# COMP6248-Reproducability-Challenge/selfsupervised-denoising

Measured on AMD Instinct MI355X. Metric: training patches/sec (64x64 gauss25 SSDN), higher is better.
Workload: dtype f16

## Files before the change

### selfsupervised-denoising_amd/csrc/api.hip

```cpp
#include "common.h"
#include <cstdarg>
#include <cstdio>
#include <cstdlib>

static thread_local char g_err[512] = "";
thread_local hipEvent_t g_ssdn_stop_event = nullptr;
thread_local bool g_ssdn_stop_used = false;
thread_local hipEvent_t g_ssdn_prof_start = nullptr, g_ssdn_prof_stop = nullptr;
thread_local bool g_ssdn_prof_used = false;

int ssdn_set_error(const char* fmt, ...) {
    va_list ap;
    va_start(ap, fmt);
    vsnprintf(g_err, sizeof(g_err), fmt, ap);
    va_end(ap);
    return -1;
}

#include <vector>
struct ProfSlot {
    bool on = false;
    std::vector<hipEvent_t> ev;
    size_t used = 0;
    double flops = 0.0, bytes = 0.0;
// ... 203 lines not shown
                }
                SSDN_CHECK_HIP(hipStreamWaitEvent(lane_s[lane], cover[src], 0));
                dirty[src][lane] = false;
            }
        }
        const bool is_mark = ops[i].type == SSDN_OP_EVENT_RECORD;
        if (!is_mark) {
            for (int d = 0; d < SSDN_NLANES; ++d) dirty[lane][d] = true;
            covered[lane] = false;
        }
        used[lane] = true;
        hipStream_t s = lane_s[lane];
        bool armed = false;
        long long armed_at = 0;
        auto arm = [&](int j) {
            if (!has_side || no_stop || j >= n) return;
            const int lj = one_lane ? 0 : ops[j].lane;
            if (lj == lane || lj < 0 || lj >= SSDN_NLANES || !((g_lane_deps[lj] >> lane) & 1)) return;
            armed_at = LS->ev_next;
            g_ssdn_stop_event = LS->ev[LS->ev_next++ % SSDN_NEVENTS];
            g_ssdn_stop_used = false;
            armed = true;
        };
        auto arm_last = [&](int j) {
            if (!has_side || no_stop || lane == 0 || armed) return;
            for (; j < n; ++j)
                if ((one_lane ? 0 : ops[j].lane) == lane && ops[j].type != SSDN_OP_EVENT_RECORD) return;
            armed_at = LS->ev_next;
            g_ssdn_stop_event = LS->ev[LS->ev_next++ % SSDN_NEVENTS];
            g_ssdn_stop_used = false;
            armed = true;
        };
        switch (ops[i].type) {
            case SSDN_OP_PACK_INPUT: {
                const bool next_conv = i + 1 < n && ops[i + 1].type == SSDN_OP_CONV && ops[i + 1].args && (one_lane ? 0 : ops[i + 1].lane) == lane;
                if (next_conv && chain_merging_on() && conv_pack_fusable((const ssdn_pack_input_args*)p, (const ssdn_conv_args*)ops[i + 1].args)) {
                    rc = launch_conv_thin((const ssdn_conv_args*)ops[i + 1].args, (const ssdn_pack_input_args*)p, s);
                    ++i;
                } else rc = launch_pack_input((const ssdn_pack_input_args*)p, s);
                break;
            }
            case SSDN_OP_CONV: {
                const int m = chain_len(ops + i, n - i, one_lane);
                if (m < 0) return -1;
                const bool pair = m <= 1 && i + 1 < n && ops[i + 1].type == SSDN_OP_CONV && ops[i + 1].args && (one_lane ? 0 : ops[i + 1].lane) == lane &&
                                  chain_merging_on() && conv_pair_fusable((const ssdn_conv_args*)p, (const ssdn_conv_args*)ops[i + 1].args);
                arm(i + (m > 1 ? m : (pair ? 2 : 1)));
                if (m > 1) { rc = launch_chain(ops + i, m, one_lane, s); i += m - 1; }
                else if (pair) { rc = launch_gemm_dma_with_next((const ssdn_conv_args*)p, (const ssdn_conv_args*)ops[i + 1].args, s); ++i; }
                else rc = launch_conv((const ssdn_conv_args*)p, s);
                break;
            }
            case SSDN_OP_POOL_FWD: rc = launch_pool_fwd((const ssdn_pool_args*)p, s); break;
            case SSDN_OP_POOL_BWD: arm(i + 1); rc = launch_pool_bwd((const ssdn_pool_args*)p, s); break;
            case SSDN_OP_UPSUM_BWD: arm(i + 1); rc = launch_upsum_bwd((const ssdn_upsum_args*)p, s); break;
            case SSDN_OP_UNROT_FWD: rc = launch_unrot_fwd((const ssdn_unrot_args*)p, s); break;
            case SSDN_OP_UNROT_BWD: arm(i + 1); rc = launch_unrot_bwd((const ssdn_unrot_args*)p, s); break;
            case SSDN_OP_WGRAD: {
                static const bool no_merge = ssdn_tuning_env("SSDN_NO_WGRAD_MERGE") != nullptr;
                {
                    const ssdn_wgrad_args* mg[WGRAD_MEGA_MAX];
                    int mm = 0;
                    while (!no_merge && mm < WGRAD_MEGA_MAX && i + mm < n && ops[i + mm].type == SSDN_OP_WGRAD && ops[i + mm].args &&
                           (one_lane ? 0 : ops[i + mm].lane) == lane && wgrad_mega_ok((const ssdn_wgrad_args*)ops[i + mm].args) &&
                           ((const ssdn_wgrad_args*)ops[i + mm].args)->mega == ((const ssdn_wgrad_args*)p)->mega)
                        mg[mm] = (const ssdn_wgrad_args*)ops[i + mm].args, ++mm;
                    if (mm > 1) { arm(i + mm); rc = launch_wgrad_mega(mg, mm, s); i += mm - 1; break; }
                }
                const ssdn_wgrad_args* items[WGRAD_MULTI_MAX];
                int m = 0;
                while (!no_merge && m < WGRAD_MULTI_MAX && i + m < n && ops[i + m].type == SSDN_OP_WGRAD && ops[i + m].args &&
                       (one_lane ? 0 : ops[i + m].lane) == lane && wgrad_mergeable((const ssdn_wgrad_args*)ops[i + m].args))
                    items[m] = (const ssdn_wgrad_args*)ops[i + m].args, ++m;
                if (m > 1) { rc = launch_wgrad_multi(items, m, s); i += m - 1; }
                else rc = launch_wgrad((const ssdn_wgrad_args*)p, s);
                break;
            }
            case SSDN_OP_WREDUCE: {
                const ssdn_wreduce_args* items[WREDUCE_MULTI_MAX];
                int m = 0;
                while (m < WREDUCE_MULTI_MAX && i + m < n && ops[i + m].type == SSDN_OP_WREDUCE && ops[i + m].args &&
                       (one_lane ? 0 : ops[i + m].lane) == lane)
                    items[m] = (const ssdn_wreduce_args*)ops[i + m].args, ++m;
                arm_last(i + m);
                rc = m > 1 ? launch_wreduce_multi(items, m, s) : launch_wreduce((const ssdn_wreduce_args*)p, s);
                i += m - 1;
                break;
            }
            case SSDN_OP_WPACK: {
                const ssdn_wpack_args* items[WPACK_MULTI_MAX];
                int m = 0;
                while (m < WPACK_MULTI_MAX && i + m < n && ops[i + m].type == SSDN_OP_WPACK && ops[i + m].args &&
                       (one_lane ? 0 : ops[i + m].lane) == lane)
                    items[m] = (const ssdn_wpack_args*)ops[i + m].args, ++m;
                rc = m > 1 ? launch_wpack_multi(items, m, s) : launch_wpack((const ssdn_wpack_args*)p, s);
                i += m - 1;
                break;
            }
            case SSDN_OP_GRAD_PACK: {
                const bool next_conv = i + 1 < n && ops[i + 1].type == SSDN_OP_CONV && ops[i + 1].args && (one_lane ? 0 : ops[i + 1].lane) == lane;
                if (next_conv && chain_merging_on() && conv_gradpack_fusable((const ssdn_grad_pack_args*)p, (const ssdn_conv_args*)ops[i + 1].args)) {
                    arm(i + 2);
                    rc = launch_gradpack_dgrad((const ssdn_grad_pack_args*)p, (const ssdn_conv_args*)ops[i + 1].args, s);
                    ++i;
                } else { arm(i + 1); rc = launch_grad_pack((const ssdn_grad_pack_args*)p, s); }
                break;
            }
            case SSDN_OP_HEAD_SSDN: rc = launch_head((const ssdn_head_args*)p, s); break;
            case SSDN_OP_HEAD_FINAL: rc = launch_head_final((const ssdn_head_final_args*)p, s); break;
            case SSDN_OP_SPATIAL_MEAN: rc = launch_spatial_mean((const ssdn_spatial_mean_args*)p, s); break;
            case SSDN_OP_MSE: rc = launch_mse((const ssdn_mse_args*)p, 0, s); break;
            case SSDN_OP_MASK_MSE: rc = launch_mse((const ssdn_mse_args*)p, 1, s); break;
            case SSDN_OP_ADAM: {
                const ssdn_wpack_args* items[ADAM_PACK_MAX];
                int m = 0;
                while (m < ADAM_PACK_MAX && i + 1 + m < n && ops[i + 1 + m].type == SSDN_OP_WPACK && ops[i + 1 + m].args &&
                       (one_lane ? 0 : ops[i + 1 + m].lane) == lane)
                    items[m] = (const ssdn_wpack_args*)ops[i + 1 + m].args, ++m;
                const bool whole_run = !(i + 1 + m < n && ops[i + 1 + m].type == SSDN_OP_WPACK);
                if (m > 0 && whole_run && adam_pack_fusable((const ssdn_adam_args*)p, items, m)) {
                    rc = launch_adam_pack((const ssdn_adam_args*)p, items, m, s);
                    i += m;
                } else rc = launch_adam((const ssdn_adam_args*)p, s);
                break;
            }
            case SSDN_OP_METRICS: rc = launch_metrics((const ssdn_metrics_args*)p, s); break;
            case SSDN_OP_NOISE: rc = launch_noise((const ssdn_noise_args*)p, s); break;
            case SSDN_OP_INPUT_GRAD: arm(i + 1); rc = launch_input_grad((const ssdn_input_grad_args*)p, s); break;
            case SSDN_OP_HEAD_VJP: rc = launch_head_vjp((const ssdn_head_vjp_args*)p, s); break;
            case SSDN_OP_MSE_VJP: rc = launch_mse_vjp((const ssdn_mse_vjp_args*)p, s); break;
            case SSDN_OP_ACCUM: rc = launch_accum((const ssdn_accum_args*)p, s); break;
            case SSDN_OP_ZERO: {
                const ssdn_zero_args* z = (const ssdn_zero_args*)p;
                if (z->bytes & 15) return ssdn_set_error("op %d: zero size must be a multiple of 16", i);
                long long n16 = z->bytes / 16;
                int g = (int)((n16 + 255) / 256);
                if (g > 2048) g = 2048;
                if (g > 0) hipLaunchKernelGGL(k_zero, dim3(g), dim3(256), 0, s, (uint4*)z->p, n16);
                break;
            }
            case SSDN_OP_EVENT_RECORD: {
                const ssdn_event_args* e = (const ssdn_event_args*)p;
                if (!e->event) return ssdn_set_error("op %d: null event", i);
                SSDN_CHECK_HIP(hipEventRecord((hipEvent_t)e->event, s));
                break;
            }
            default: return ssdn_set_error("op %d: unknown type %d", i, ops[i].type);
        }
        if (armed) {
            if (g_ssdn_stop_used && !rc) { cover[lane] = g_ssdn_stop_event; covered[lane] = true; cover_at[lane] = armed_at; }
            g_ssdn_stop_event = nullptr;
        }
        if (rc) {
            char tmp[400];
            snprintf(tmp, sizeof(tmp), "%s", g_err);
            return ssdn_set_error("op %d (type %d): %s", i, ops[i].type, tmp);
        }
    }
    for (int l = 1; l < SSDN_NLANES; ++l) {
        if (!used[l]) continue;
        if (!cover_live(l)) {
            cover[l] = LS->ev[LS->ev_next++ % SSDN_NEVENTS];
            SSDN_CHECK_HIP(hipEventRecord(cover[l], lane_s[l]));
        }
        SSDN_CHECK_HIP(hipStreamWaitEvent(lane_s[0], cover[l], 0));
    }
// ... 41 lines not shown
```

### selfsupervised-denoising_amd/csrc/common.h

```cpp
#pragma once
#include <hip/hip_runtime.h>
#include <hip/hip_ext.h>
#include <stdint.h>
#include "../../include/ssdn_hip.h"
#include <cstdlib>

#if defined(SSDN_TUNING)
static inline const char* ssdn_tuning_env(const char* name) { return std::getenv(name); }
#else
static inline const char* ssdn_tuning_env(const char*) { return nullptr; }
#endif

typedef _Float16 h16;
typedef _Float16 half8 __attribute__((ext_vector_type(8)));
typedef _Float16 half4 __attribute__((ext_vector_type(4)));
typedef _Float16 half2v __attribute__((ext_vector_type(2)));
typedef __bf16 bf16x8 __attribute__((ext_vector_type(8)));
typedef unsigned short u16x8 __attribute__((ext_vector_type(8)));
typedef unsigned short u16x4 __attribute__((ext_vector_type(4)));
typedef float f32x16 __attribute__((ext_vector_type(16)));
typedef float f32x4 __attribute__((ext_vector_type(4)));

#define LRELU_SLOPE 0.1f

// ... 31 lines not shown
}
static __device__ __forceinline__ float bf_lo(unsigned w) { return __uint_as_float(w << 16); }
static __device__ __forceinline__ float bf_hi(unsigned w) { return __uint_as_float(w & 0xffff0000u); }
static __device__ __forceinline__ float f16_lo(unsigned w) { return (float)__builtin_bit_cast(f16x2_t, w)[0]; }
static __device__ __forceinline__ float f16_hi(unsigned w) { return (float)__builtin_bit_cast(f16x2_t, w)[1]; }
#define SSDN_BUFFER_RSRC_FLAGS 0x00020000
static __device__ __forceinline__ u16x8 ld_b8(const unsigned short* p) { return *reinterpret_cast<const u16x8*>(p); }
static __device__ __forceinline__ void st_b8(unsigned short* p, u16x8 v) { *reinterpret_cast<u16x8*>(p) = v; }
static __device__ __forceinline__ u16x4 ld_b4(const unsigned short* p) { return *reinterpret_cast<const u16x4*>(p); }
static __device__ __forceinline__ void st_b4(unsigned short* p, u16x4 v) { *reinterpret_cast<u16x4*>(p) = v; }
static __device__ __forceinline__ u16x8 zero_b8() {
    u16x8 z;
#pragma unroll
    for (int i = 0; i < 8; ++i) z[i] = 0;
    return z;
}

static __device__ __forceinline__ half8 zero_h8() {
    half8 z;
#pragma unroll
    for (int i = 0; i < 8; ++i) z[i] = (h16)0.f;
    return z;
}

extern thread_local hipEvent_t g_ssdn_stop_event;
extern thread_local bool g_ssdn_stop_used;
extern thread_local hipEvent_t g_ssdn_prof_start, g_ssdn_prof_stop;
extern thread_local bool g_ssdn_prof_used;
#define SSDN_LAUNCH(kernel, grid, block, lds, stream, ...)                                                                       \
    do {                                                                                                                         \
        if (g_ssdn_stop_event) {                                                                                                 \
            hipExtLaunchKernelGGL(kernel, grid, block, lds, stream, nullptr, g_ssdn_stop_event, 0, __VA_ARGS__);                 \
            g_ssdn_stop_used = true;                                                                                             \
        } else if (g_ssdn_prof_start) {                                                                                          \
            hipExtLaunchKernelGGL(kernel, grid, block, lds, stream, g_ssdn_prof_start, g_ssdn_prof_stop, 0, __VA_ARGS__);        \
            g_ssdn_prof_start = nullptr;                                                                                         \
            g_ssdn_prof_used = true;                                                                                             \
        } else hipLaunchKernelGGL(kernel, grid, block, lds, stream, __VA_ARGS__);                                                \
    } while (0)

#define SSDN_MAX_DEVICES_ATTR 16
static inline int ssdn_current_device_slot() {
    int dev = 0;
    if (hipGetDevice(&dev) != hipSuccess || dev < 0) dev = 0;
    return dev % SSDN_MAX_DEVICES_ATTR;
}

void prof_begin(int kind, hipStream_t s);
void prof_end(int kind, hipStream_t s, double flops, double bytes);

int launch_conv(const ssdn_conv_args* a, hipStream_t s);
int launch_wgrad(const ssdn_wgrad_args* a, hipStream_t s);
bool wgrad_mergeable(const ssdn_wgrad_args* a);
int launch_wgrad_multi(const ssdn_wgrad_args* const* items, int n, hipStream_t s);
#define WGRAD_MEGA_MAX 64
int wgrad_mega_ok(const ssdn_wgrad_args* a);
int launch_wgrad_mega(const ssdn_wgrad_args* const* ops, int n, hipStream_t s);
int launch_pack_input(const ssdn_pack_input_args* a, hipStream_t s);
int launch_pool_fwd(const ssdn_pool_args* a, hipStream_t s);
int launch_pool_bwd(const ssdn_pool_args* a, hipStream_t s);
int launch_upsum_bwd(const ssdn_upsum_args* a, hipStream_t s);
int launch_unrot_fwd(const ssdn_unrot_args* a, hipStream_t s);
int launch_unrot_bwd(const ssdn_unrot_args* a, hipStream_t s);
int launch_wreduce(const ssdn_wreduce_args* a, hipStream_t s);
int launch_wpack(const ssdn_wpack_args* a, hipStream_t s);
#define WPACK_MULTI_MAX 24
int launch_wpack_multi(const ssdn_wpack_args* const* items, int n, hipStream_t s);
#define WREDUCE_MULTI_MAX 32
#define WGRAD_MULTI_MAX 32
int launch_wreduce_multi(const ssdn_wreduce_args* const* items, int n, hipStream_t s);
int launch_grad_pack(const ssdn_grad_pack_args* a, hipStream_t s);
int launch_head(const ssdn_head_args* a, hipStream_t s);
int launch_head_impulse(const ssdn_head_args* a, hipStream_t s);
int launch_head_final(const ssdn_head_final_args* a, hipStream_t s);
int launch_spatial_mean(const ssdn_spatial_mean_args* a, hipStream_t s);
int launch_mse(const ssdn_mse_args* a, int masked, hipStream_t s);
int launch_head_vjp(const ssdn_head_vjp_args* a, hipStream_t s);
int launch_head_vjp_impulse(const ssdn_head_vjp_args* a, hipStream_t s);
int launch_mse_vjp(const ssdn_mse_vjp_args* a, hipStream_t s);
int launch_adam(const ssdn_adam_args* a, hipStream_t s);
#define ADAM_PACK_MAX 24
int adam_pack_fusable(const ssdn_adam_args* a, const ssdn_wpack_args* const* items, int n);
int launch_adam_pack(const ssdn_adam_args* a, const ssdn_wpack_args* const* items, int n, hipStream_t s);
int launch_metrics(const ssdn_metrics_args* a, hipStream_t s);
int launch_accum(const ssdn_accum_args* a, hipStream_t s);
int launch_noise(const ssdn_noise_args* a, hipStream_t s);
int launch_input_grad(const ssdn_input_grad_args* a, hipStream_t s);
int conv_lds_bytes(const ssdn_conv_args* a);
int conv_validate(const ssdn_conv_args* a);
int chain_len(const ssdn_op* ops, int n, bool any_lane);
int launch_chain(const ssdn_op* ops, int n, bool any_lane, hipStream_t s);
bool chain_merging_on();
bool conv_dma_eligible(const ssdn_conv_args* a, bool any_size);
int conv_dma_lds_bytes(int mt);
bool conv_signs(const ssdn_conv_args* a);
bool gemm_dma_signs(const ssdn_conv_args* a);
bool conv_dma_signs(const ssdn_conv_args* a);
bool conv_fuses_urot(const ssdn_conv_args* a);
bool conv_fuses_unrot(const ssdn_conv_args* a);
bool conv_fuses_upsum(const ssdn_conv_args* a);
bool conv_fuses_pool(const ssdn_conv_args* a);
int launch_conv_dma(const ssdn_conv_args* a, hipStream_t s);
bool conv_thin_eligible(const ssdn_conv_args* a);
bool conv_thin_fuses_pack(const ssdn_pack_input_args* pk, const ssdn_conv_args* a);
int launch_conv_thin(const ssdn_conv_args* a, const ssdn_pack_input_args* pk, hipStream_t s);
bool conv_pack_fusable(const ssdn_pack_input_args* pk, const ssdn_conv_args* a);
bool gradpack_dgrad_fusable(const ssdn_grad_pack_args* gp, const ssdn_conv_args* a);
int launch_gradpack_dgrad(const ssdn_grad_pack_args* gp, const ssdn_conv_args* a, hipStream_t s);
bool conv_gradpack_fusable(const ssdn_grad_pack_args* gp, const ssdn_conv_args* a);
bool gemm_dma_eligible(const ssdn_conv_args* a);
int gemm_dma_lds_bytes(const ssdn_conv_args* a);
int launch_gemm_dma(const ssdn_conv_args* a, hipStream_t s);
bool gemm_dma_fuses_next(const ssdn_conv_args* a, const ssdn_conv_args* b);
int launch_gemm_dma_with_next(const ssdn_conv_args* a, const ssdn_conv_args* b, hipStream_t s);
bool conv_pair_fusable(const ssdn_conv_args* a, const ssdn_conv_args* b);
extern "C" int ssdn_device_cus(void);
int wgrad_lds_bytes(const ssdn_wgrad_args* a);
```

### selfsupervised-denoising_amd/csrc/elementwise.hip

```cpp
#include "common.h"

#define EW_BLOCK 256
static inline int ew_grid(long long n) {
    long long g = (n + EW_BLOCK - 1) / EW_BLOCK;
    return (int)(g < 1 ? 1 : g);
}

__global__ void k_pack_input(ssdn_pack_input_args a) {
    const unsigned idx = blockIdx.x * blockDim.x + threadIdx.x;
    const int H = a.H, W = a.W;
    long long total = (long long)a.R * a.B * H * W;
    if (idx >= total) return;
    int j = idx % W;
    int i = (idx / W) % H;
    int nb = idx / (unsigned)(W * H);
    int r = nb / a.B, b = nb % a.B;
    int sy, sx;
    switch (r) {
        case 0: sy = i; sx = j; break;
        case 1: sy = j; sx = W - 1 - i; break;
        case 2: sy = H - 1 - i; sx = W - 1 - j; break;
        default: sy = H - 1 - j; sx = i; break;
    }
    h16* d = (h16*)a.dst.p + (long long)idx * a.dst.cs + a.dst.co;
    for (int c0 = 0; c0 < a.cpad; c0 += 8) {
        half8 v = zero_h8();
#pragma unroll
        for (int c = 0; c < 8; ++c)
            if (c0 + c < a.C) v[c] = (h16)a.src[(((long long)b * a.C + c0 + c) * H + sy) * W + sx];
        st_h8(d + c0, v);
    }
}
int launch_pack_input(const ssdn_pack_input_args* a, hipStream_t s) {
    if (a->R == 4 && a->H != a->W) return ssdn_set_error("pack_input: blind-spot rotation needs square images");
    long long n = (long long)a->R * a->B * a->H * a->W;
    if (n >= (1ll << 31)) return ssdn_set_error("pack_input: too many elements for 32-bit indexing");
    hipLaunchKernelGGL(k_pack_input, dim3(ew_grid(n)), dim3(EW_BLOCK), 0, s, *a);
    return 0;
}

__global__ void k_pool_fwd(ssdn_pool_args a) {
    const unsigned idx = blockIdx.x * blockDim.x + threadIdx.x;
    const int C8 = a.C >> 3, Ho = a.H >> 1, Wo = a.W >> 1;
    long long total = (long long)a.N * Ho * Wo * C8;
    if (idx >= total) return;
    int c = (idx % C8) * 8;
    const unsigned p = idx / C8;
    int j = p % Wo;
    int i = (p / Wo) % Ho;
    int n = p / (unsigned)(Wo * Ho);
    const h16* src = (const h16*)a.act.p + a.act.co + c;
    int r0 = a.shifted ? 2 * i - 1 : 2 * i;
    const bool padrow = a.shifted && r0 < 0;
    float m[8];
    unsigned win[8];
#pragma unroll
    for (int q = 0; q < 8; ++q) { m[q] = padrow ? 0.f : -65504.f; win[q] = 4u; }
#pragma unroll
    for (int dr = 0; dr < 2; ++dr) {
        int y = r0 + dr;
        if (y < 0) continue;
#pragma unroll
        for (int dc = 0; dc < 2; ++dc) {
            half8 v = ld_h8(src + (((long long)n * a.H + y) * a.W + 2 * j + dc) * a.act.cs);
#pragma unroll
            for (int q = 0; q < 8; ++q) {
                const float f = (float)v[q];
                if (f > m[q] || (!padrow && dr == 0 && dc == 0)) win[q] = (unsigned)(2 * dr + dc);
                m[q] = fmaxf(m[q], f);
            }
        }
    }
    half8 o;
#pragma unroll
    for (int q = 0; q < 8; ++q) o[q] = (h16)m[q];
    st_h8((h16*)a.pooled.p + a.pooled.co + c + (((long long)n * Ho + i) * Wo + j) * a.pooled.cs, o);
    if (a.route) {
        unsigned r = 0;
#pragma unroll
        for (int q = 0; q < 8; ++q) r |= (win[q] | (m[q] > 0.f ? 8u : 0u)) << (4 * q);
        ((unsigned*)a.route)[idx] = r;
    }
}
// ... 416 lines not shown
        t1.bstart[i] = b1;
        t2.bstart[i] = b2;
        if (a->nslabs > WR_GROUP) {
            t1.gx[i] = ew_grid(stride / 4);
            b1 += t1.gx[i] * ((a->nslabs + WR_GROUP - 1) / WR_GROUP);
            t2.step[i] = WR_GROUP;
        } else {
            t1.gx[i] = 0;
            t2.step[i] = 1;
        }
        t1.step[i] = t2.step[i];
        t2.gx[i] = t1.gx[i];
        if (a->Kpad & 3) return ssdn_set_error("wreduce: Kpad must be a multiple of 4");
        b2 += ew_grid(stride / 4 + a->M);
    }
    t1.bstart[n] = b1;
    t2.bstart[n] = b2;
    if (b1 > 0) hipLaunchKernelGGL(k_wreduce_partial_multi, dim3(b1), dim3(EW_BLOCK), 0, s, t1);
    if (b2 > 0) SSDN_LAUNCH(k_wreduce_multi, dim3(b2), dim3(EW_BLOCK), 0, s, t2);
    return 0;
}

int launch_wreduce(const ssdn_wreduce_args* a, hipStream_t s) {
    long long stride = (long long)a->ntaps * a->Mpad * a->Kpad;
    int step = 1;
    if (a->nslabs > WR_GROUP) {
        int groups = (a->nslabs + WR_GROUP - 1) / WR_GROUP;
        hipLaunchKernelGGL(k_wreduce_partial, dim3(ew_grid(stride / 4), groups), dim3(EW_BLOCK), 0, s, (float*)a->slab, stride, a->nslabs);
        step = WR_GROUP;
    }
    if (a->Kpad & 3) return ssdn_set_error("wreduce: Kpad must be a multiple of 4");
    long long n = stride / 4 + a->M;
    SSDN_LAUNCH(k_wreduce, dim3(ew_grid(n)), dim3(EW_BLOCK), 0, s, *a, step);
    return 0;
}

__global__ void k_accum(ssdn_accum_args a) {
    const long long i = (long long)blockIdx.x * blockDim.x + threadIdx.x;
    if (i < a.n) a.dst[i] = __fadd_rn(a.dst[i], a.src[i]);
}
int launch_accum(const ssdn_accum_args* a, hipStream_t s) {
    if (!a->dst || !a->src || a->n < 0) return ssdn_set_error("accum: dst and src must be given, n >= 0");
    if (a->n > 0) hipLaunchKernelGGL(k_accum, dim3(ew_grid(a->n)), dim3(EW_BLOCK), 0, s, *a);
    return 0;
}

struct AdamIn { float g, m, v, p; };
static __device__ __forceinline__ AdamIn adam_load(const ssdn_adam_args& a, long long i) { return AdamIn{a.g[i], a.m[i], a.v[i], a.p[i]}; }
static __device__ __forceinline__ float adam_apply(const ssdn_adam_args& a, long long i, const AdamIn& q, float inv_bc2s, float step) {
    const float g = q.g * a.gscale;
    const float m = __fmaf_rn(a.b1, q.m, __fmul_rn(1.f - a.b1, g));
    const float v = __fmaf_rn(a.b2, q.v, __fmul_rn(__fmul_rn(1.f - a.b2, g), g));
    a.m[i] = m;
    a.v[i] = v;
    const float den = __fmaf_rn(sqrtf(v), inv_bc2s, a.eps);
    const float pn = __fsub_rn(q.p, __fdiv_rn(__fmul_rn(step, m), den));
    a.p[i] = pn;
    return pn;
}
static __device__ __forceinline__ float adam_elem(const ssdn_adam_args& a, long long i, float inv_bc2s, float step) {
    return adam_apply(a, i, adam_load(a, i), inv_bc2s, step);
}
__global__ void k_adam(ssdn_adam_args a) {
    long long i = (long long)blockIdx.x * blockDim.x + threadIdx.x;
    long long stride = (long long)gridDim.x * blockDim.x;
    float inv_bc2s = 1.f / sqrtf(a.bc2);
    float step = a.lr / a.bc1;
    for (; i < a.n; i += stride) adam_elem(a, i, inv_bc2s, step);
}
#define AP_TM 8
#define AP_TK 48
struct AdamPackTable {
    ssdn_adam_args a;
    ssdn_wpack_args e[ADAM_PACK_MAX];
    long long w_off[ADAM_PACK_MAX];
    int bstart[ADAM_PACK_MAX + 1];
    int tiles_k[ADAM_PACK_MAX];
    long long gap_start[ADAM_PACK_MAX + 2];
    long long gap_end[ADAM_PACK_MAX + 2];
    int gap_bstart[ADAM_PACK_MAX + 3];
    int n, ngaps;
};
template <int NT>
static __device__ __forceinline__ void adam_pack_tile(const AdamPackTable& t, int j, int tile, float* lds, float inv_bc2s, float step) {
    const ssdn_adam_args& a = t.a;
    const ssdn_wpack_args& w = t.e[j];
    const int tk = t.tiles_k[j];
    const int mo0 = (tile / tk) * AP_TM, k0 = (tile % tk) * AP_TK;
    const int tid = threadIdx.x;
    constexpr int TOTAL = AP_TM * AP_TK * NT, NIT = (TOTAL + EW_BLOCK - 1) / EW_BLOCK, BATCH = NIT < 7 ? NIT : 7;
#pragma unroll
    for (int it0 = 0; it0 < NIT; it0 += BATCH) {
        AdamIn q[BATCH];
        long long idx[BATCH];
        bool ok[BATCH];
#pragma unroll
        for (int u = 0; u < BATCH; ++u) {
            const int e = tid + (it0 + u) * EW_BLOCK;
            const int mo = e / (AP_TK * NT), r = e - mo * (AP_TK * NT);
            const int kk = r / NT, tp = r - kk * NT;
            ok[u] = it0 + u < NIT && e < TOTAL && mo0 + mo < w.M && k0 + kk < w.cin;
            idx[u] = ok[u] ? t.w_off[j] + ((long long)(mo0 + mo) * w.cin + k0 + kk) * NT + tp : t.w_off[j];
            q[u] = adam_load(a, idx[u]);
        }
#pragma unroll
        for (int u = 0; u < BATCH; ++u) {
            const int e = tid + (it0 + u) * EW_BLOCK;
            if (it0 + u >= NIT || e >= TOTAL) continue;
            const int mo = e / (AP_TK * NT), r = e - mo * (AP_TK * NT);
            const int kk = r / NT, tp = r - kk * NT;
            lds[(tp * AP_TM + mo) * (AP_TK + 1) + kk] = ok[u] ? adam_apply(a, idx[u], q[u], inv_bc2s, step) : 0.f;
        }
    }
    __syncthreads();
    for (int e = tid; e < NT * AP_TM * AP_TK; e += EW_BLOCK) {
        const int tp = e / (AP_TM * AP_TK), r = e - tp * (AP_TM * AP_TK);
        const int mo = r / AP_TK, kk = r - mo * AP_TK;
        const int m = mo0 + mo, k = k0 + kk;
        if (m >= w.M || k >= w.cin) continue;
        const float pn = lds[(tp * AP_TM + mo) * (AP_TK + 1) + kk];
        ((h16*)w.wf)[((long long)tp * w.Mpad_f + m) * w.Ktot + k] = (h16)pn;
        if (w.wfc) ((h16*)w.wfc)[wpack_cm(tp, m, k, w.Mpad_f, w.Ktot)] = (h16)pn;
    }
    if (w.wd) {
        for (int e = tid; e < NT * AP_TK * AP_TM; e += EW_BLOCK) {
            const int tp = e / (AP_TK * AP_TM), r = e - tp * (AP_TK * AP_TM);
            const int kk = r / AP_TM, mo = r - kk * AP_TM;
            const int m = mo0 + mo, k = k0 + kk;
            if (m >= w.M || k >= w.cin || k >= w.Mpad_d || m >= w.Kd) continue;
            const float pn = lds[(tp * AP_TM + mo) * (AP_TK + 1) + kk];
            ((unsigned short*)w.wd)[((long long)tp * w.Mpad_d + k) * w.Kd + m] = f2bf(pn);
            if (w.wdc) ((unsigned short*)w.wdc)[wpack_cm(tp, k, m, w.Mpad_d, w.Kd)] = f2bf(pn);
        }
    }
}
__global__ void k_adam_pack(AdamPackTable t) {
    __shared__ float lds[9 * AP_TM * (AP_TK + 1)];
    const ssdn_adam_args& a = t.a;
    const float inv_bc2s = 1.f / sqrtf(a.bc2);
    const float step = a.lr / a.bc1;
    const int b = blockIdx.x;
    if (b < t.bstart[t.n]) {
        int j = 0;
        while (j + 1 < t.n && b >= t.bstart[j + 1]) ++j;
        if (t.e[j].ntaps == 9) adam_pack_tile<9>(t, j, b - t.bstart[j], lds, inv_bc2s, step);
        else adam_pack_tile<1>(t, j, b - t.bstart[j], lds, inv_bc2s, step);
    } else {
        int g = 0;
        while (g + 1 < t.ngaps && b >= t.gap_bstart[g + 1]) ++g;
        const long long first = t.gap_start[g] + (long long)(b - t.gap_bstart[g]) * (EW_BLOCK * 4) + threadIdx.x;
#pragma unroll
        for (int u = 0; u < 4; ++u) {
            const long long i = first + u * EW_BLOCK;
            if (i < t.gap_end[g]) adam_elem(a, i, inv_bc2s, step);
        }
    }
}
int adam_pack_fusable(const ssdn_adam_args* a, const ssdn_wpack_args* const* items, int n) {
    if (n < 1 || n > ADAM_PACK_MAX) return 0;
    long long prev = -1;
    for (int i = 0; i < n; ++i) {
        const ssdn_wpack_args* w = items[i];
        const long long off = w->w - a->p;
        if (w->w < a->p || off + (long long)w->M * w->cin * w->ntaps > a->n || off <= prev) return 0;
        if (w->c0 + w->c1_real != w->cin || (w->ntaps != 1 && w->ntaps != 9)) return 0;
        prev = off;
    }
    return 1;
}
int launch_adam_pack(const ssdn_adam_args* a, const ssdn_wpack_args* const* items, int n, hipStream_t s) {
    AdamPackTable t;
    t.a = *a;
    t.n = n;
    int blocks = 0, ng = 0;
    long long pos = 0;
    auto gap = [&](long long start, long long end) {
        if (end <= start) return;
        t.gap_start[ng] = start; t.gap_end[ng] = end;
        ++ng;
    };
    for (int i = 0; i < n; ++i) {
        t.e[i] = *items[i];
        t.w_off[i] = items[i]->w - a->p;
        t.bstart[i] = blocks;
        t.tiles_k[i] = (items[i]->cin + AP_TK - 1) / AP_TK;
        blocks += ((items[i]->M + AP_TM - 1) / AP_TM) * t.tiles_k[i];
        gap(pos, t.w_off[i]);
        pos = t.w_off[i] + (long long)items[i]->M * items[i]->cin * items[i]->ntaps;
    }
    t.bstart[n] = blocks;
    gap(pos, a->n);
    t.ngaps = ng;
    for (int g = 0; g < ng; ++g) {
        t.gap_bstart[g] = blocks;
        blocks += (int)((t.gap_end[g] - t.gap_start[g] + EW_BLOCK * 4 - 1) / (EW_BLOCK * 4));
    }
    t.gap_bstart[ng] = blocks;
    if (blocks > 0) hipLaunchKernelGGL(k_adam_pack, dim3(blocks), dim3(EW_BLOCK), 0, s, t);
    return 0;
}
int launch_adam(const ssdn_adam_args* a, hipStream_t s) {
    int g = ew_grid(a->n);
    if (g > 2048) g = 2048;
    hipLaunchKernelGGL(k_adam, dim3(g), dim3(EW_BLOCK), 0, s, *a);
    return 0;
}

struct Ph4 { unsigned v[4]; };
static __device__ __forceinline__ Ph4 philox4x32_10(unsigned c0, unsigned c1, unsigned c2, unsigned c3, unsigned k0, unsigned k1) {
#pragma unroll
    for (int r = 0; r < 10; ++r) {
        const unsigned hi0 = __umulhi(0xD2511F53u, c0), lo0 = 0xD2511F53u * c0;
        const unsigned hi1 = __umulhi(0xCD9E8D57u, c2), lo1 = 0xCD9E8D57u * c2;
        const unsigned n0 = hi1 ^ c1 ^ k0, n2 = hi0 ^ c3 ^ k1;
        c0 = n0; c1 = lo1; c2 = n2; c3 = lo0;
        k0 += 0x9E3779B9u; k1 += 0xBB67AE85u;
    }
    Ph4 o;
    o.v[0] = c0; o.v[1] = c1; o.v[2] = c2; o.v[3] = c3;
    return o;
}
static __device__ __forceinline__ float u01(unsigned x) { return (float)(x >> 8) * (1.f / 16777216.f) + (0.5f / 16777216.f); }
enum { NS_INPUT = 0, NS_REF = 1, NS_PARAM = 2, NS_COORD = 3, NS_PARAM_REF = 4 };
static __device__ __forceinline__ float noise_apply(const ssdn_noise_args& a, float clean, float param, unsigned e, unsigned stream) {
    const Ph4 r = philox4x32_10(e, stream, (unsigned)a.offset, (unsigned)(a.offset >> 32), (unsigned)a.seed, (unsigned)(a.seed >> 32));
    float v;
    if (a.style == 0) {
        const float z = sqrtf(-2.f * __logf(u01(r.v[0]))) * __cosf(6.28318530718f * u01(r.v[1]));
        v = clean + param * z;
    } else {
        const float u = u01(r.v[0]);
        float pk = 0.36787944117f, cdf = pk;
        int k = 0;
        while (u > cdf && k < 16) { ++k; pk /= (float)k; cdf += pk; }
        v = (clean * param + (float)k) / param;
    }
    if (a.clip) v = fminf(fmaxf(v, 0.f), 1.f);
    return v;
}
static __device__ __forceinline__ float noise_param(const ssdn_noise_args& a, int bc, unsigned stream) {
    if (a.p_lo == a.p_hi) return a.p_lo;
    const Ph4 r = philox4x32_10((unsigned)bc, stream, (unsigned)a.offset, (unsigned)(a.offset >> 32), (unsigned)a.seed, (unsigned)(a.seed >> 32));
    return a.p_lo + (a.p_hi - a.p_lo) * u01(r.v[0]);
}
static __device__ __forceinline__ int n2v_pick(int c, int r, int size, float u) {
    const int lo = c - r < 0 ? c - r : 0, hi = c + r < size - 1 ? c + r : size - 1;
    int span = hi - lo - (c >= lo && c < hi ? 1 : 0);
    if (span < 1) span = 1;
    int k = (int)(u * (float)span);
    if (k >= span) k = span - 1;
    int v = lo + k;
    if (c >= lo && c < hi && v >= c) ++v;
    if (v < 0) v += size;
    if (v >= size) v = size - 1;
    return v;
}
__global__ void k_noise(ssdn_noise_args a) {
    const unsigned idx = blockIdx.x * blockDim.x + threadIdx.x;
    const int H = a.H, W = a.W, HW = H * W;
    if (idx >= (unsigned)(a.B * HW)) return;
    const int x = idx % W, y = (idx / W) % H, b = idx / HW;
    const unsigned char* u8 = (const unsigned char*)a.clean_u8;
    bool blind = false;
    int rx = x, ry = y;
    if (a.n2v_box > 0) {
        const int box = a.n2v_box, n1 = H / box, i = x / box, j = y / box, cell = i * n1 + j;
        const unsigned ce = (unsigned)(b * (W / box) * n1 + cell);
        const Ph4 r = philox4x32_10(ce, NS_COORD, (unsigned)a.offset, (unsigned)(a.offset >> 32), (unsigned)a.seed, (unsigned)(a.seed >> 32));
        int c0 = i * box + (int)(u01(r.v[0]) * (float)box), c1 = j * box + (int)(u01(r.v[1]) * (float)box);
        c0 = c0 > i * box + box - 1 ? i * box + box - 1 : c0;
        c1 = c1 > j * box + box - 1 ? j * box + box - 1 : c1;
        if (c0 == x && c1 == y) {
            blind = true;
            rx = n2v_pick(c0, a.n2v_radius, W, u01(r.v[2]));
            ry = n2v_pick(c1, a.n2v_radius, H, u01(r.v[3]));
            a.coords[((long long)b * (W / box) * n1 + cell) * 2 + 0] = c0;
            a.coords[((long long)b * (W / box) * n1 + cell) * 2 + 1] = c1;
        }
    }
    for (int c = 0; c < a.C; ++c) {
        const int bc = b * a.C + c;
// ... 94 lines not shown
```

Baseline: 20720.

## Fuse weight-gradient slab reduction into the Adam+weight-pack tail kernel

Adds a fused kernel that reduces the per-slab weight and bias gradient partials directly inside the Adam update and bf16 weight-pack tiles, replacing a separate wreduce launch followed by adam_pack. This removes one kernel launch and a full write-then-read round trip of the reduced gradient buffer. The fused table is too large for kernel arguments, so it is cached in device memory, keyed by the table contents. In exchange there is more per-tile work, heavier register use, and extra host-side table building and comparison on every launch.

```diff
diff --git a/selfsupervised-denoising_amd/csrc/api.hip b/selfsupervised-denoising_amd/csrc/api.hip
--- a/selfsupervised-denoising_amd/csrc/api.hip
+++ b/selfsupervised-denoising_amd/csrc/api.hip
@@ -309,6 +309,22 @@
                 while (m < WREDUCE_MULTI_MAX && i + m < n && ops[i + m].type == SSDN_OP_WREDUCE && ops[i + m].args &&
                        (one_lane ? 0 : ops[i + m].lane) == lane)
                     items[m] = (const ssdn_wreduce_args*)ops[i + m].args, ++m;
+                const int ia = i + m;
+                if (ia < n && ops[ia].type == SSDN_OP_ADAM && ops[ia].args && (one_lane ? 0 : ops[ia].lane) == lane) {
+                    const ssdn_wpack_args* packs[ADAM_PACK_MAX];
+                    int pm = 0;
+                    while (pm < ADAM_PACK_MAX && ia + 1 + pm < n && ops[ia + 1 + pm].type == SSDN_OP_WPACK && ops[ia + 1 + pm].args &&
+                           (one_lane ? 0 : ops[ia + 1 + pm].lane) == lane)
+                        packs[pm] = (const ssdn_wpack_args*)ops[ia + 1 + pm].args, ++pm;
+                    const bool whole_run = !(ia + 1 + pm < n && ops[ia + 1 + pm].type == SSDN_OP_WPACK);
+                    static const bool no_tail = ssdn_tuning_env("SSDN_NO_TAIL_FUSION") != nullptr;
+                    if (!no_tail && pm > 0 && whole_run && wreduce_adam_pack_fusable(items, m, (const ssdn_adam_args*)ops[ia].args, packs, pm)) {
+                        arm_last(ia + 1 + pm);
+                        rc = launch_wreduce_adam_pack(items, m, (const ssdn_adam_args*)ops[ia].args, packs, pm, s);
+                        i = ia + pm;
+                        break;
+                    }
+                }
                 arm_last(i + m);
                 rc = m > 1 ? launch_wreduce_multi(items, m, s) : launch_wreduce((const ssdn_wreduce_args*)p, s);
                 i += m - 1;
diff --git a/selfsupervised-denoising_amd/csrc/common.h b/selfsupervised-denoising_amd/csrc/common.h
--- a/selfsupervised-denoising_amd/csrc/common.h
+++ b/selfsupervised-denoising_amd/csrc/common.h
@@ -137,6 +137,8 @@
 #define ADAM_PACK_MAX 24
 int adam_pack_fusable(const ssdn_adam_args* a, const ssdn_wpack_args* const* items, int n);
 int launch_adam_pack(const ssdn_adam_args* a, const ssdn_wpack_args* const* items, int n, hipStream_t s);
+int wreduce_adam_pack_fusable(const ssdn_wreduce_args* const* reds, int nr, const ssdn_adam_args* a, const ssdn_wpack_args* const* items, int n);
+int launch_wreduce_adam_pack(const ssdn_wreduce_args* const* reds, int nr, const ssdn_adam_args* a, const ssdn_wpack_args* const* items, int n, hipStream_t s);
 int launch_metrics(const ssdn_metrics_args* a, hipStream_t s);
 int launch_accum(const ssdn_accum_args* a, hipStream_t s);
 int launch_noise(const ssdn_noise_args* a, hipStream_t s);
diff --git a/selfsupervised-denoising_amd/csrc/elementwise.hip b/selfsupervised-denoising_amd/csrc/elementwise.hip
--- a/selfsupervised-denoising_amd/csrc/elementwise.hip
+++ b/selfsupervised-denoising_amd/csrc/elementwise.hip
@@ -1,4 +1,7 @@
 #include "common.h"
+#include <cstring>
+#include <mutex>
+#include <vector>
 
 #define EW_BLOCK 256
 static inline int ew_grid(long long n) {
@@ -581,37 +584,8 @@
     int n, ngaps;
 };
 template <int NT>
-static __device__ __forceinline__ void adam_pack_tile(const AdamPackTable& t, int j, int tile, float* lds, float inv_bc2s, float step) {
-    const ssdn_adam_args& a = t.a;
-    const ssdn_wpack_args& w = t.e[j];
-    const int tk = t.tiles_k[j];
-    const int mo0 = (tile / tk) * AP_TM, k0 = (tile % tk) * AP_TK;
+static __device__ __forceinline__ void adam_pack_store(const ssdn_wpack_args& w, int mo0, int k0, const float* lds) {
     const int tid = threadIdx.x;
-    constexpr int TOTAL = AP_TM * AP_TK * NT, NIT = (TOTAL + EW_BLOCK - 1) / EW_BLOCK, BATCH = NIT < 7 ? NIT : 7;
-#pragma unroll
-    for (int it0 = 0; it0 < NIT; it0 += BATCH) {
-        AdamIn q[BATCH];
-        long long idx[BATCH];
-        bool ok[BATCH];
-#pragma unroll
-        for (int u = 0; u < BATCH; ++u) {
-            const int e = tid + (it0 + u) * EW_BLOCK;
-            const int mo = e / (AP_TK * NT), r = e - mo * (AP_TK * NT);
-            const int kk = r / NT, tp = r - kk * NT;
-            ok[u] = it0 + u < NIT && e < TOTAL && mo0 + mo < w.M && k0 + kk < w.cin;
-            idx[u] = ok[u] ? t.w_off[j] + ((long long)(mo0 + mo) * w.cin + k0 + kk) * NT + tp : t.w_off[j];
-            q[u] = adam_load(a, idx[u]);
-        }
-#pragma unroll
-        for (int u = 0; u < BATCH; ++u) {
-            const int e = tid + (it0 + u) * EW_BLOCK;
-            if (it0 + u >= NIT || e >= TOTAL) continue;
-            const int mo = e / (AP_TK * NT), r = e - mo * (AP_TK * NT);
-            const int kk = r / NT, tp = r - kk * NT;
-            lds[(tp * AP_TM + mo) * (AP_TK + 1) + kk] = ok[u] ? adam_apply(a, idx[u], q[u], inv_bc2s, step) : 0.f;
-        }
-    }
-    __syncthreads();
     for (int e = tid; e < NT * AP_TM * AP_TK; e += EW_BLOCK) {
         const int tp = e / (AP_TM * AP_TK), r = e - tp * (AP_TM * AP_TK);
         const int mo = r / AP_TK, kk = r - mo * AP_TK;
@@ -632,6 +606,40 @@
             if (w.wdc) ((unsigned short*)w.wdc)[wpack_cm(tp, k, m, w.Mpad_d, w.Kd)] = f2bf(pn);
         }
     }
+}
+template <int NT>
+static __device__ __forceinline__ void adam_pack_tile(const AdamPackTable& t, int j, int tile, float* lds, float inv_bc2s, float step) {
+    const ssdn_adam_args& a = t.a;
+    const ssdn_wpack_args& w = t.e[j];
+    const int tk = t.tiles_k[j];
+    const int mo0 = (tile / tk) * AP_TM, k0 = (tile % tk) * AP_TK;
+    const int tid = threadIdx.x;
+    constexpr int TOTAL = AP_TM * AP_TK * NT, NIT = (TOTAL + EW_BLOCK - 1) / EW_BLOCK, BATCH = NIT < 7 ? NIT : 7;
+#pragma unroll
+    for (int it0 = 0; it0 < NIT; it0 += BATCH) {
+        AdamIn q[BATCH];
+        long long idx[BATCH];
+        bool ok[BATCH];
+#pragma unroll
+        for (int u = 0; u < BATCH; ++u) {
+            const int e = tid + (it0 + u) * EW_BLOCK;
+            const int mo = e / (AP_TK * NT), r = e - mo * (AP_TK * NT);
+            const int kk = r / NT, tp = r - kk * NT;
+            ok[u] = it0 + u < NIT && e < TOTAL && mo0 + mo < w.M && k0 + kk < w.cin;
+            idx[u] = ok[u] ? t.w_off[j] + ((long long)(mo0 + mo) * w.cin + k0 + kk) * NT + tp : t.w_off[j];
+            q[u] = adam_load(a, idx[u]);
+        }
+#pragma unroll
+        for (int u = 0; u < BATCH; ++u) {
+            const int e = tid + (it0 + u) * EW_BLOCK;
+            if (it0 + u >= NIT || e >= TOTAL) continue;
+            const int mo = e / (AP_TK * NT), r = e - mo * (AP_TK * NT);
+            const int kk = r / NT, tp = r - kk * NT;
+            lds[(tp * AP_TM + mo) * (AP_TK + 1) + kk] = ok[u] ? adam_apply(a, idx[u], q[u], inv_bc2s, step) : 0.f;
+        }
+    }
+    __syncthreads();
+    adam_pack_store<NT>(w, mo0, k0, lds);
 }
 __global__ void k_adam_pack(AdamPackTable t) {
     __shared__ float lds[9 * AP_TM * (AP_TK + 1)];
@@ -667,8 +675,7 @@
     }
     return 1;
 }
-int launch_adam_pack(const ssdn_adam_args* a, const ssdn_wpack_args* const* items, int n, hipStream_t s) {
-    AdamPackTable t;
+static int adam_pack_table(const ssdn_adam_args* a, const ssdn_wpack_args* const* items, int n, AdamPackTable& t) {
     t.a = *a;
     t.n = n;
     int blocks = 0, ng = 0;
@@ -695,7 +702,303 @@
         blocks += (int)((t.gap_end[g] - t.gap_start[g] + EW_BLOCK * 4 - 1) / (EW_BLOCK * 4));
     }
     t.gap_bstart[ng] = blocks;
+    return blocks;
+}
+int launch_adam_pack(const ssdn_adam_args* a, const ssdn_wpack_args* const* items, int n, hipStream_t s) {
+    AdamPackTable t;
+    const int blocks = adam_pack_table(a, items, n, t);
     if (blocks > 0) hipLaunchKernelGGL(k_adam_pack, dim3(blocks), dim3(EW_BLOCK), 0, s, t);
+    return 0;
+}
+
+struct TailTable {
+    AdamPackTable ap;
+    ssdn_wreduce_args r[WREDUCE_MULTI_MAX];
+    int lay_r[WREDUCE_MULTI_MAX];
+    int lay_first[ADAM_PACK_MAX + 1];
+    const float* lay_inv[ADAM_PACK_MAX];
+    int lay_acc[ADAM_PACK_MAX];
+    int bias_r[WREDUCE_MULTI_MAX];
+    long long bias_off[WREDUCE_MULTI_MAX];
+    int gap_bfirst[ADAM_PACK_MAX + 3];
+    int nr;
+};
+#define TAIL_G __attribute__((address_space(1)))
+static __device__ __forceinline__ f32x4 tail_ld4(const float* p) { return *(const TAIL_G f32x4*)p; }
+static __device__ __forceinline__ float tail_ld1(const float* p) { return *(const TAIL_G float*)p; }
+template <int NT>
+static __device__ __forceinline__ void tail_slab_sums(const ssdn_wreduce_args& r, int mo0, int k0, int Mlay, int Clay, float* lds) {
+    constexpr int TQ = NT == 9 ? 4 : 1;
+    const int mlo = max(mo0, r.m_off), mhi = min(min(mo0 + AP_TM, Mlay), r.m_off + r.M);
+    const int clo = max(k0, r.c_off), chi = min(min(k0 + AP_TK, Clay), r.c_off + r.cin);
+    if (mlo >= mhi || clo >= chi) return;
+    const int q0 = (clo - r.c_off) >> 2, nq = ((chi - r.c_off + 3) >> 2) - q0, nrow = mhi - mlo;
+    const int items = NT * nrow * nq;
+    const long long st = (long long)r.ntaps * r.Mpad * r.Kpad;
+    const int nslabs = r.nslabs;
+    for (int base = 0; base < items; base += TQ * EW_BLOCK) {
+        unsigned off[TQ];
+        int pos[TQ], c[TQ];
+#pragma unroll
+        for (int u = 0; u < TQ; ++u) {
+            const int e = base + (int)threadIdx.x + u * EW_BLOCK;
+            const bool on = e < items;
+            const int q = on ? e % nq : 0, rw = on ? (e / nq) % nrow : 0, tp = on ? e / (nq * nrow) : 0;
+            const int m = mlo + rw;
+            off[u] = (unsigned)((tp * r.Mpad + (m - r.m_off)) * r.Kpad + (q0 + q) * 4);
+            c[u] = on ? r.c_off + (q0 + q) * 4 : -8;
+            pos[u] = (tp * AP_TM + (m - mo0)) * (AP_TK + 1) - k0;
+        }
+        f32x4 tot[TQ], grp[TQ];
+#pragma unroll
+        for (int u = 0; u < TQ; ++u) tot[u] = f32x4{0.f, 0.f, 0.f, 0.f};
+        for (int s0 = 0; s0 < nslabs; s0 += WR_GROUP) {
+            const int s1 = s0 + WR_GROUP < nslabs ? s0 + WR_GROUP : nslabs;
+#pragma unroll
+            for (int u = 0; u < TQ; ++u) grp[u] = f32x4{0.f, 0.f, 0.f, 0.f};
+            for (int s = s0; s < s1; s += 8) {
+                const int nv = s1 - s < 8 ? s1 - s : 8;
+                f32x4 v[TQ][8];
+#pragma unroll
+                for (int k = 0; k < 8; ++k) {
+                    const float* sb = r.slab + (long long)(s + (k < nv ? k : nv - 1)) * st;
+#pragma unroll
+                    for (int u = 0; u < TQ; ++u) v[u][k] = tail_ld4(sb + off[u]);
+                }
+#pragma unroll
+                for (int k = 0; k < 8; ++k) {
+                    if (k < nv) {
+#pragma unroll
+                        for (int u = 0; u < TQ; ++u) grp[u] += v[u][k];
+                    }
+                }
+            }
+            if (nslabs > WR_GROUP) {
+#pragma unroll
+                for (int u = 0; u < TQ; ++u) tot[u] += grp[u];
+            } else {
+#pragma unroll
+                for (int u = 0; u < TQ; ++u) tot[u] = grp[u];
+            }
+        }
+#pragma unroll
+        for (int u = 0; u < TQ; ++u) {
+            const float t4[4] = {tot[u][0], tot[u][1], tot[u][2], tot[u][3]};
+#pragma unroll
+            for (int j = 0; j < 4; ++j)
+                if (c[u] + j >= clo && c[u] + j < chi) lds[pos[u] + c[u] + j] = t4[j];
+        }
+    }
+}
+template <int NT>
+static __device__ __forceinline__ void tail_tile(const TailTable& T, const ssdn_adam_args& a, int j, int tile, float* lds, float inv_bc2s, float step) {
+    const AdamPackTable& t = T.ap;
+    const ssdn_wpack_args& w = t.e[j];
+    const int tk = t.tiles_k[j];
+    const int mo0 = (tile / tk) * AP_TM, k0 = (tile % tk) * AP_TK;
+    const int tid = threadIdx.x;
+    const int r0 = T.lay_first[j], r1 = T.lay_first[j + 1];
+    const bool acc = r1 > r0 && T.lay_acc[j];
+    float* const gout = const_cast<float*>(a.g);
+    constexpr int TOTAL = AP_TM * AP_TK * NT, NIT = (TOTAL + EW_BLOCK - 1) / EW_BLOCK, BATCH = NIT < 5 ? NIT : 5;
+    auto place = [&](int it, long long& idx, int& slot) {
+        const int e = tid + it * EW_BLOCK;
+        const int mo = e / (AP_TK * NT), r = e - mo * (AP_TK * NT);
+        const int kk = r / NT, tp = r - kk * NT;
+        const bool ok = it < NIT && e < TOTAL && mo0 + mo < w.M && k0 + kk < w.cin;
+        idx = ok ? t.w_off[j] + ((long long)(mo0 + mo) * w.cin + k0 + kk) * NT + tp : t.w_off[j];
+        slot = it < NIT && e < TOTAL ? (tp * AP_TM + mo) * (AP_TK + 1) + kk : -1;
+        return ok;
+    };
+    auto fetch = [&](int it, AdamIn& q) {
+        const int e = tid + it * EW_BLOCK;
+        const int mo = e / (AP_TK * NT), kk = (e - mo * (AP_TK * NT)) / NT;
+        const int m = mo0 + mo, c = k0 + kk;
+        long long idx;
+        int slot;
+        const bool ok = place(it, idx, slot);
+        bool cov = false;
+        for (int ri = r0; ri < r1; ++ri) {
+            const ssdn_wreduce_args& r_ = T.r[T.lay_r[ri]];
+            cov = cov || (ok && m >= r_.m_off && m < r_.m_off + r_.M && c >= r_.c_off && c < r_.c_off + r_.cin);
+        }
+        q.g = (!cov || acc) ? a.g[idx] : 0.f;
+        q.m = a.m[idx]; q.v = a.v[idx]; q.p = a.p[idx];
+        return cov;
+    };
+    AdamIn q[BATCH];
+    unsigned cov = 0;
+#pragma unroll
+    for (int u = 0; u < BATCH; ++u) cov |= fetch(u, q[u]) ? 1u << u : 0u;
+    float inv = 1.f;
+    if (r1 > r0) {
+        if (T.lay_inv[j]) inv = tail_ld1(T.lay_inv[j]);
+        for (int ri = r0; ri < r1; ++ri) tail_slab_sums<NT>(T.r[T.lay_r[ri]], mo0, k0, w.M, w.cin, lds);
+        __syncthreads();
+    }
+#pragma unroll
+    for (int it0 = 0; it0 < NIT; it0 += BATCH) {
+        if (it0 > 0) {
+            cov = 0;
+#pragma unroll
+            for (int u = 0; u < BATCH; ++u) cov |= fetch(it0 + u, q[u]) ? 1u << u : 0u;
+        }
+#pragma unroll
+        for (int u = 0; u < BATCH; ++u) {
+            long long idx;
+            int slot;
+            const bool ok = place(it0 + u, idx, slot);
+            if (slot < 0) continue;
+            if ((cov >> u) & 1) {
+                const float g = __fmul_rn(lds[slot], inv);
+                q[u].g = acc ? __fadd_rn(q[u].g, g) : g;
+                gout[idx] = q[u].g;
+            }
+            lds[slot] = ok ? adam_apply(a, idx, q[u], inv_bc2s, step) : 0.f;
+        }
+    }
+    __syncthreads();
+    adam_pack_store<NT>(w, mo0, k0, lds);
+}
+__global__ void __launch_bounds__(EW_BLOCK, 2) k_wreduce_adam_pack(const TailTable* __restrict__ Tp, ssdn_adam_args a) {
+    __shared__ float lds[9 * AP_TM * (AP_TK + 1)];
+    const TailTable& T = *Tp;
+    const AdamPackTable& t = T.ap;
+    const float inv_bc2s = 1.f / sqrtf(a.bc2);
+    const float step = a.lr / a.bc1;
+    const int b = blockIdx.x;
+    if (b < t.bstart[t.n]) {
+        int j = 0;
+        while (j + 1 < t.n && b >= t.bstart[j + 1]) ++j;
+        if (t.e[j].ntaps == 9) tail_tile<9>(T, a, j, b - t.bstart[j], lds, inv_bc2s, step);
+        else tail_tile<1>(T, a, j, b - t.bstart[j], lds, inv_bc2s, step);
+    } else {
+        int g = 0;
+        while (g + 1 < t.ngaps && b >= t.gap_bstart[g + 1]) ++g;
+        const long long first = t.gap_start[g] + (long long)(b - t.gap_bstart[g]) * (EW_BLOCK * 4) + threadIdx.x;
+        float* const gout = const_cast<float*>(a.g);
+#pragma unroll
+        for (int u = 0; u < 4; ++u) {
+            const long long i = first + u * EW_BLOCK;
+            if (i >= t.gap_end[g]) continue;
+            AdamIn q = adam_load(a, i);
+            for (int bi = T.gap_bfirst[g]; bi < T.gap_bfirst[g + 1]; ++bi) {
+                const ssdn_wreduce_args& r = T.r[T.bias_r[bi]];
+                const long long m = i - T.bias_off[bi];
+                if (m < 0 || m >= r.M) continue;
+                float acc = 0.f;
+                int s = 0;
+                for (; s + 16 <= r.nslabs; s += 16) {
+                    float v[16];
+#pragma unroll
+                    for (int k = 0; k < 16; ++k) v[k] = tail_ld1(r.bslab + (long long)(s + k) * r.Mpad + m);
+#pragma unroll
+                    for (int k = 0; k < 16; ++k) acc += v[k];
+                }
+                for (; s < r.nslabs; ++s) acc += tail_ld1(r.bslab + (long long)s * r.Mpad + m);
+                const float gb = __fmul_rn(acc, r.inv_scale ? tail_ld1(r.inv_scale) : 1.f);
+                q.g = r.accumulate ? __fadd_rn(q.g, gb) : gb;
+                gout[i] = q.g;
+            }
+            adam_apply(a, i, q, inv_bc2s, step);
+        }
+    }
+}
+static int tail_table(const ssdn_wreduce_args* const* reds, int nr, const ssdn_adam_args* a, const ssdn_wpack_args* const* items, int n, TailTable& T, int* blocks) {
+    if (nr < 1 || nr > WREDUCE_MULTI_MAX || !a->g || !adam_pack_fusable(a, items, n)) return 0;
+    memset((void*)&T, 0, sizeof(T));
+    *blocks = adam_pack_table(a, items, n, T.ap);
+    memset((void*)&T.ap.a, 0, sizeof(T.ap.a));
+    const AdamPackTable& t = T.ap;
+    T.nr = nr;
+    int lay_of[WREDUCE_MULTI_MAX], gap_of[WREDUCE_MULTI_MAX];
+    for (int i = 0; i < nr; ++i) {
+        const ssdn_wreduce_args* r = reds[i];
+        T.r[i] = *r;
+        if (r->tapblock || (r->Kpad & 3) || r->nslabs < 1 || !r->slab || !r->gw || r->M < 1 || r->cin < 1 || r->M > r->Mpad || r->cin > r->Kpad ||
+            r->m_off < 0 || r->c_off < 0 || (long long)r->ntaps * r->Mpad * r->Kpad >= (1ll << 31))
+            return 0;
+        lay_of[i] = -1;
+        for (int j = 0; j < n; ++j)
+            if (r->gw == a->g + t.w_off[j]) lay_of[i] = j;
+        if (lay_of[i] < 0) return 0;
+        const ssdn_wpack_args& w = t.e[lay_of[i]];
+        if (r->ntaps != w.ntaps || r->cin_full != w.cin || r->m_off + r->M > w.M || r->c_off + r->cin > w.cin) return 0;
+        gap_of[i] = -1;
+        if (r->gb) {
+            if (!r->bslab) return 0;
+            const long long off = (r->gb + r->m_off) - a->g;
+            for (int g = 0; g < t.ngaps; ++g)
+                if (r->gb + r->m_off >= a->g && off >= t.gap_start[g] && off + r->M <= t.gap_end[g]) gap_of[i] = g;
+            if (gap_of[i] < 0) return 0;
+        }
+        for (int k = 0; k < i; ++k) {
+            const ssdn_wreduce_args* o = reds[k];
+            if (lay_of[k] == lay_of[i] && r->m_off < o->m_off + o->M && o->m_off < r->m_off + r->M && r->c_off < o->c_off + o->cin && o->c_off < r->c_off + r->cin)
+                return 0;
+            if (r->gb && o->gb && r->gb + r->m_off < o->gb + o->m_off + o->M && o->gb + o->m_off < r->gb + r->m_off + r->M) return 0;
+        }
+    }
+    int pos = 0;
+    for (int j = 0; j < n; ++j) {
+        T.lay_first[j] = pos;
+        for (int i = 0; i < nr; ++i) {
+            if (lay_of[i] != j) continue;
+            if (pos == T.lay_first[j]) { T.lay_inv[j] = reds[i]->inv_scale; T.lay_acc[j] = reds[i]->accumulate != 0; }
+            else if (T.lay_inv[j] != reds[i]->inv_scale || T.lay_acc[j] != (reds[i]->accumulate != 0)) return 0;
+            T.lay_r[pos++] = i;
+        }
+    }
+    T.lay_first[n] = pos;
+    pos = 0;
+    for (int g = 0; g < t.ngaps; ++g) {
+        T.gap_bfirst[g] = pos;
+        for (int i = 0; i < nr; ++i) {
+            if (gap_of[i] != g) continue;
+            T.bias_off[pos] = (reds[i]->gb + reds[i]->m_off) - a->g;
+            T.bias_r[pos++] = i;
+        }
+    }
+    T.gap_bfirst[t.ngaps] = pos;
+    return 1;
+}
+int wreduce_adam_pack_fusable(const ssdn_wreduce_args* const* reds, int nr, const ssdn_adam_args* a, const ssdn_wpack_args* const* items, int n) {
+    TailTable T;
+    int blocks = 0;
+    return tail_table(reds, nr, a, items, n, T, &blocks);
+}
+namespace {
+struct TailCache {
+    std::vector<char> key;
+    TailTable* dev;
+    int device;
+};
+std::vector<TailCache> g_tail_cache;
+std::mutex g_tail_mutex;
+}
+int launch_wreduce_adam_pack(const ssdn_wreduce_args* const* reds, int nr, const ssdn_adam_args* a, const ssdn_wpack_args* const* items, int n, hipStream_t s) {
+    TailTable T;
+    int blocks = 0;
+    if (!tail_table(reds, nr, a, items, n, T, &blocks)) return ssdn_set_error("wreduce + adam + wpack: the run cannot be fused");
+    int dev = 0;
+    SSDN_CHECK_HIP(hipGetDevice(&dev));
+    TailTable* dtab = nullptr;
+    {
+        std::lock_guard<std::mutex> lock(g_tail_mutex);
+        for (const TailCache& c : g_tail_cache)
+            if (c.device == dev && !memcmp(c.key.data(), &T, sizeof(T))) { dtab = c.dev; break; }
+        if (!dtab) {
+            if (g_tail_cache.size() >= 64) {
+                SSDN_CHECK_HIP(hipDeviceSynchronize());
+                SSDN_CHECK_HIP(hipFree(g_tail_cache.front().dev));
+                g_tail_cache.erase(g_tail_cache.begin());
+            }
+            SSDN_CHECK_HIP(hipMalloc((void**)&dtab, sizeof(T)));
+            SSDN_CHECK_HIP(hipMemcpy(dtab, &T, sizeof(T), hipMemcpyHostToDevice));
+            g_tail_cache.push_back({std::vector<char>((const char*)&T, (const char*)&T + sizeof(T)), dtab, dev});
+        }
+    }
+    if (blocks > 0) SSDN_LAUNCH(k_wreduce_adam_pack, dim3(blocks), dim3(EW_BLOCK), 0, s, (const TailTable*)dtab, *a);
     return 0;
 }
 int launch_adam(const ssdn_adam_args* a, hipStream_t s) {
```

New measurement: 20780 (median of 2 runs). No clear change (+0.3%).
